# GBATZOLIS/conditional_score_diffusion

Measured on AMD Instinct MI355X. Metric: images/sec for 1000-step PC sampling, ddpm_paired_SR3 score net of celebA_SR3_160 (BASELINE configs[1]), 160x160, higher is better.
Workload: dtype f16x3 (every operand carried as hi + lo fp16 = 22 significand bits, 3 MFMAs per product, f32 accumulate; f32-class: the per-op test tolerance is the f32 kernel's, network error 1.9e-6 vs the reference); 1 GPU; BASELINE configs[1]: celebA_SR3_160 (ddpm_paired_SR3, nf=96, ch_mult (1,1,2,2,3,3), attn 20/10/5), 1000-step PC (reverse_diffusion + langevin, snr 0.15), batch 64 per GPU, random-init weights, synthetic LR inputs; images_per_gpu=64, global_batch=64, noise=on-device Philox4x32-10, precision_mode=fp16x3

## Files before the change

### conditional_score_diffusion_amd/csrc/conv_f16_q.hip

```cpp
#include <stdlib.h>
#include <type_traits>

#include "conv_f16_kernel.h"

namespace csd {

typedef float floatx4q __attribute__((ext_vector_type(4)));
typedef unsigned int uint4q __attribute__((ext_vector_type(4)));

#define C16Q_THREADS 256

__device__ __forceinline__ double dpp_row16_sum(double v) {
#define CSD_DPP_STEP(CTRL)                                                                                   \
  {                                                                                                          \
    const int lo = __builtin_amdgcn_mov_dpp(__double2loint(v), CTRL, 0xF, 0xF, true);                        \
    const int hi = __builtin_amdgcn_mov_dpp(__double2hiint(v), CTRL, 0xF, 0xF, true);                        \
    v += __hiloint2double(hi, lo);                                                                           \
  }
  CSD_DPP_STEP(0xB1)
  CSD_DPP_STEP(0x4E)
  CSD_DPP_STEP(0x124)
  CSD_DPP_STEP(0x128)
#undef CSD_DPP_STEP
  return v;
}
__device__ __forceinline__ float dpp_row16_sum(float v) {
#define CSD_DPP_STEP_F(CTRL) v += __int_as_float(__builtin_amdgcn_mov_dpp(__float_as_int(v), CTRL, 0xF, 0xF, true));
  CSD_DPP_STEP_F(0xB1)
  CSD_DPP_STEP_F(0x4E)
  CSD_DPP_STEP_F(0x124)
  CSD_DPP_STEP_F(0x128)
#undef CSD_DPP_STEP_F
  return v;
}

typedef int int8q __attribute__((ext_vector_type(8)));

template <int MQ, int NS, bool MASK, int PWC, int S, int NTQ, bool F8, bool UP4 = false, bool RAW = false>
__global__ __launch_bounds__(C16Q_THREADS, 2) void conv_f16_q_kernel(const void* __restrict__ g_hi,
                                                                    const void* __restrict__ g_lo,
                                                                    const char* __restrict__ g_wpack,
                                                                    const Conv16KArgs k) {
  static_assert(!UP4 || (S == 1 && !F8), "the phase form is the stride-1 Upsample conv (a resampling conv: full split)");
  static_assert(!RAW || (NS == 2 && !F8), "the fp32-source form splits into two fp16 planes");
  constexpr int TAPS = UP4 ? 4 : 9, KS = UP4 ? 2 : 3, KCS = 2;
  constexpr int LO = 32 * KCS;
  constexpr int PSB = 32 * KCS * NS + 16;
  constexpr int NPIX = 2 * MQ * 16;
  constexpr int SPP = 2 * NS * KCS;
  constexpr int NU0 = (S == 2) ? ((NS == 2) ? 10 : 5) : ((NS == 2) ? 7 : 4);
  constexpr int NU = RAW ? 2 * ((NU0 + 1) / 2) : NU0;
  constexpr int rstride = PWC * PSB;
  constexpr int WSTEP = NTQ * NS * 1024;
  constexpr int GC = 32 * NTQ, HC = 16 * NTQ;
  extern __shared__ __attribute__((aligned(16))) char smem16[];

  const int tid = threadIdx.x;
#ifdef CSD_C16_TIMING
  int ts_n = 0;
#define Q_TSTAMP() do { if (k.a.dbg && tid == 0 && blockIdx.x < 4095 && ts_n < 8) k.a.dbg[blockIdx.x * 8 + ts_n++] = clock64(); } while (0)
#else
#define Q_TSTAMP() do { } while (0)
#endif
  Q_TSTAMP();
  const int lane = tid & 63;
  const int wave = __builtin_amdgcn_readfirstlane(tid >> 6);
  const int mi = wave >> 1, ni = wave & 1;
  const int l16 = lane & 15, kq = lane >> 4;

  int w;
  {
    const int bid = blockIdx.x, nb = k.nblocks;
    const int xcd = bid & 7, slot = bid >> 3;
    const int q = nb >> 3, r = nb & 7;
    w = (xcd < r ? xcd * (q + 1) : r * (q + 1) + (xcd - r) * q) + slot;
  }
  const int ng = w % k.n_groups;
  const int tile4 = w / k.n_groups;
  const int ph = UP4 ? (tile4 & 3) : 0, pa = ph >> 1, pb = ph & 1;
  const int tile = UP4 ? (tile4 >> 2) : tile4;
  const int tile_y = tile / k.tiles_x;
  const int ov0 = tile_y * k.TH, ox0 = (tile - tile_y * k.tiles_x) * k.TW;
  const int Py = UP4 ? 1 - pa : ((S == 2) ? 0 : 1), Px = UP4 ? 1 - pb : ((S == 2) ? 0 : 1);
  const int prow0 = ov0 * S - Py, pcol0 = ox0 * S - Px;
  const int EH = (S == 2) ? k.IH : k.OH, EW = (S == 2) ? k.IW : k.OW;
  const int Cin = k.C0;
  const int npatch = k.PH * k.PW;
  const int patch_bytes = k.PH * PWC * PSB;
  int* const otab = reinterpret_cast<int*>(smem16 + patch_bytes);
  int* const btab = otab + NPIX;
  int* const vtab = btab + NPIX;
  int* const stab = vtab + NPIX;
  int* const dtab = stab + npatch;

  for (int m = tid; m < NPIX; m += C16Q_THREADS) {
    const int ty = m / k.TW, tx = m - ty * k.TW;
    const int ov = ov0 + ty, ox = ox0 + tx;
    const bool mv = (m < k.TH * k.TW) && (ov < k.B * k.OH) && (ox < k.OW);
    const int b = ov / k.OH, oy = ov - b * k.OH;
    unsigned vb = 0;
#pragma unroll
    for (int r = 0; r < KS; ++r) {
      const int iy = oy * S + r - Py, ix = ox * S + r - Px;
      vb |= ((mv && iy >= 0 && iy < EH) ? 1u : 0u) << r;
      vb |= ((mv && ix >= 0 && ix < EW) ? 1u : 0u) << (3 + r);
    }
    otab[m] = mv ? (UP4 ? (ov - ov0) * 4 * k.OW + 2 * ox : (ov - ov0) * k.OW + ox) : -1;
    btab[m] = mv ? b : 0;
    vtab[m] = (int)vb;
  }
  for (int pix = tid; pix < npatch; pix += C16Q_THREADS) {
    const int pr = pix / k.PW, pc = pix - pr * k.PW;
    const int vr = prow0 + pr, col = pcol0 + pc;
    const int img_lo = MASK ? 0 : (ov0 / k.OH) * EH;
    const int img_hi = MASK ? k.B * EH : img_lo + EH;
    const bool in = vr >= img_lo && vr < img_hi && col >= 0 && col < EW;
    const int sb = vr / EH, sr = vr - sb * EH;
    stab[pix] = in ? (sb * k.IH + (sr >> k.up)) * k.IW + (col >> k.up) : -1;
    dtab[pix] = (pr * PWC + pc) * PSB;
  }
  int base[MQ];
#pragma unroll
  for (int j = 0; j < MQ; ++j) {
    const int m = (mi * MQ + j) * 16 + l16;
    const int ty = m / k.TW, tx = m - ty * k.TW;
    base[j] = (m < k.TH * k.TW) ? ty * S * rstride + tx * S * PSB + kq * 16 : kq * 16;
  }
  __syncthreads();
  Q_TSTAMP();
  unsigned vbits[MQ];
  if (MASK) {
#pragma unroll
    for (int j = 0; j < MQ; ++j) vbits[j] = (unsigned)vtab[(mi * MQ + j) * 16 + l16];
  }

  const int total4 = RAW ? npatch * 2 * KCS : npatch * SPP;
  auto raw_load = [&](int e, int cb, int half) -> float4 {
    float4 v = make_float4(0.f, 0.f, 0.f, 0.f);
    if (e < total4) {
      const int pix = e / (2 * KCS), grp = e - pix * (2 * KCS);
      const int sp = stab[pix];
      if (sp >= 0) v = gload4f(static_cast<const float*>(g_hi) + (size_t)sp * Cin + cb + grp * 8 + half * 4);
    }
    return v;
  };
  auto raw_store = [&](int e, const float4& a, const float4& b) {
    if (e >= total4) return;
    const int pix = e / (2 * KCS), grp = e - pix * (2 * KCS);
    const float v[8] = {a.x, a.y, a.z, a.w, b.x, b.y, b.z, b.w};
    half8 h, l;
#pragma unroll
    for (int j = 0; j < 8; ++j) {
      h[j] = (_Float16)v[j];
      l[j] = (_Float16)(v[j] - (float)h[j]);
    }
    *reinterpret_cast<half8*>(smem16 + dtab[pix] + grp * 16) = h;
    *reinterpret_cast<half8*>(smem16 + dtab[pix] + LO + grp * 16) = l;
  };
  auto slot_load = [&](int e, int cb) -> float4 {
    float4 v = make_float4(0.f, 0.f, 0.f, 0.f);
    if (e < total4) {
      const int pix = e / SPP, sub = e - pix * SPP;
      const int sp = stab[pix];
      if (sp >= 0) {
        const int pl = sub / (2 * KCS), rest = sub - pl * (2 * KCS);
        const _Float16* plane = static_cast<const _Float16*>((NS == 2 && pl) ? g_lo : g_hi);
        v = gload4f(reinterpret_cast<const float*>(plane + (size_t)sp * Cin + cb + rest * 8));
      }
    }
    return v;
  };
  auto slot_store = [&](int e, const float4& v) {
    if (e >= total4) return;
    const int pix = e / SPP, sub = e - pix * SPP;
    const int pl = sub / (2 * KCS), rest = sub - pl * (2 * KCS);
    *reinterpret_cast<float4*>(smem16 + dtab[pix] + pl * LO + rest * 16) = v;
  };

  constexpr int BR = UP4 ? 2 : (NTQ == 1 && !F8 ? 9 : 3);
  const int nk32 = Cin / 32;
  const char* wstep = g_wpack + ((size_t)((UP4 ? ph * k.n_groups * 2 : 0) + ng * 2 + ni) * nk32 * TAPS) * WSTEP + lane * 16;
  constexpr int NP = F8 ? 1 : NS;
  half8 wreg[BR][NTQ][NP];
#pragma unroll
  for (int q = 0; q < BR - 1; ++q)
#pragma unroll
    for (int t = 0; t < NTQ; ++t)
#pragma unroll
      for (int p = 0; p < NP; ++p) wreg[q][t][p] = gload_h8(wstep + (size_t)q * WSTEP + (t * NS + p) * 1024);
  wstep += (size_t)(BR - 2) * WSTEP;
  const char* const w8base = g_wpack + ((size_t)(ng * 2 + ni) * nk32 * TAPS + (kq >> 1)) * WSTEP + (lane & 31) * 32 + 1024;
  int8q w8[1][NTQ];
  auto load_w8 = [&](int buf, int step) {
#pragma unroll
    for (int t = 0; t < NTQ; ++t) {
      const uint4q a = *reinterpret_cast<const uint4q*>(w8base + (size_t)step * WSTEP + t * NS * 1024);
      const uint4q c = *reinterpret_cast<const uint4q*>(w8base + (size_t)step * WSTEP + t * NS * 1024 + 16);
      w8[buf][t] = int8q{(int)a.x, (int)a.y, (int)a.z, (int)a.w, (int)c.x, (int)c.y, (int)c.z, (int)c.w};
    }
  };
  if constexpr (F8) load_w8(0, 0);
  int base8[MQ];
#pragma unroll
  for (int j = 0; j < MQ; ++j) base8[j] = base[j] - kq * 16 + LO + (kq & 1) * 32;

  floatx4q acc[MQ][NTQ];
#pragma unroll
  for (int j = 0; j < MQ; ++j)
#pragma unroll
    for (int t = 0; t < NTQ; ++t) acc[j][t] = floatx4q{0.f, 0.f, 0.f, 0.f};

  {
    float4 v0[NU];
    if constexpr (RAW) {
#pragma unroll
      for (int j = 0; j < NU; ++j) v0[j] = raw_load((j >> 1) * C16Q_THREADS + tid, 0, j & 1);
#pragma unroll
      for (int j = 0; j < NU; j += 2) raw_store((j >> 1) * C16Q_THREADS + tid, v0[j], v0[j + 1]);
    } else {
#pragma unroll
      for (int j = 0; j < NU; ++j) v0[j] = slot_load(j * C16Q_THREADS + tid, 0);
#pragma unroll
      for (int j = 0; j < NU; ++j) slot_store(j * C16Q_THREADS + tid, v0[j]);
    }
  }
  __syncthreads();
  Q_TSTAMP();

  const int nstage = nk32;
  for (int stg = 0; stg < nstage; ++stg) {
    const bool more = stg + 1 < nstage;
    float4 sv[NU];
    if (more) {
#pragma unroll
      for (int j = 0; j < NU; ++j)
        sv[j] = RAW ? raw_load((j >> 1) * C16Q_THREADS + tid, (stg + 1) * 32, j & 1) : slot_load(j * C16Q_THREADS + tid, (stg + 1) * 32);
    }
#ifdef CSD_Q_RING
    constexpr int RING = CSD_Q_RING;
#else
    constexpr int RING = 2;
#endif
    half8 preg[RING][NP];
    auto load_frag = [&](int q) {
      const int tap_ = q / MQ, j_ = q % MQ;
      const char* p = smem16 + base[j_] + (tap_ / KS) * rstride + (tap_ % KS) * PSB;
#pragma unroll
      for (int pl = 0; pl < NP; ++pl) preg[q % RING][pl] = *reinterpret_cast<const half8*>(p + pl * LO);
    };
#pragma unroll
    for (int q = 0; q < RING - 1; ++q) load_frag(q);
#pragma unroll
    for (int tap = 0; tap < TAPS; ++tap) {
      const int bc = tap % BR, bn = (tap + BR - 1) % BR;
      const int r = tap / KS, sx = tap % KS;
      wstep += WSTEP;
#ifndef CSD_Q_ABLATE
#define CSD_Q_ABLATE 0
#endif
#pragma unroll
      for (int t = 0; t < ((CSD_Q_ABLATE & 1) ? 1 : NTQ); ++t)
#pragma unroll
        for (int p = 0; p < NP; ++p) wreg[bn][t][p] = gload_h8(wstep + (t * NS + p) * 1024);

#pragma unroll
      for (int j = 0; j < MQ; ++j) {
        const int q = tap * MQ + j;
        if (q + RING - 1 < TAPS * MQ) load_frag(q + RING - 1);
        __builtin_amdgcn_sched_barrier(0);
        half8 b[NP];
        const bool v = !MASK || (((vbits[j] >> r) & 1u) && ((vbits[j] >> (3 + sx)) & 1u));
#pragma unroll
        for (int pl = 0; pl < NP; ++pl) {
          b[pl] = preg[q % RING][pl];
          if (MASK && !v) {
#pragma unroll
            for (int e = 0; e < 8; ++e) b[pl][e] = (_Float16)0.f;
          }
        }
#pragma unroll
        for (int t = 0; t < NTQ; ++t) {
          if constexpr (NS == 2 && !F8) {
            acc[j][t] = __builtin_amdgcn_mfma_f32_16x16x32_f16(wreg[bc][t][1], b[0], acc[j][t], 0, 0, 0);
            acc[j][t] = __builtin_amdgcn_mfma_f32_16x16x32_f16(wreg[bc][t][0], b[1], acc[j][t], 0, 0, 0);
          }
          acc[j][t] = __builtin_amdgcn_mfma_f32_16x16x32_f16(wreg[bc][t][0], b[0], acc[j][t], 0, 0, 0);
        }
        __builtin_amdgcn_sched_barrier(0);
      }
      if constexpr (F8) {
        if (tap % 2 == 1 || tap == TAPS - 1) {
          const int t0 = tap % 2 == 1 ? tap - 1 : tap;
          const bool pair = t0 + 1 < TAPS;
          const int t1 = pair ? t0 + 1 : t0;
          const int o0 = (t0 / KS) * rstride + (t0 % KS) * PSB, o1 = (t1 / KS) * rstride + (t1 % KS) * PSB;
          const int off = (kq >> 1) ? o1 : o0;
          constexpr int wb = 0;
#pragma unroll
          for (int j = 0; j < MQ; ++j) {
            const char* xp = smem16 + base8[j] + off;
            const uint4q a = *reinterpret_cast<const uint4q*>(xp);
            const uint4q c = *reinterpret_cast<const uint4q*>(xp + 16);
            bool ok = pair || (kq >> 1) == 0;
            if (MASK) {
              const int tt = (kq >> 1) ? t1 : t0;
              ok = ok && ((vbits[j] >> (tt / KS)) & 1u) && ((vbits[j] >> (3 + tt % KS)) & 1u);
            }
            const int8q b8 = int8q{ok ? (int)a.x : 0, ok ? (int)a.y : 0, ok ? (int)a.z : 0, ok ? (int)a.w : 0,
                                   ok ? (int)c.x : 0, ok ? (int)c.y : 0, ok ? (int)c.z : 0, ok ? (int)c.w : 0};
#pragma unroll
            for (int t = 0; t < NTQ; ++t)
              acc[j][t] = __builtin_amdgcn_mfma_scale_f32_16x16x128_f8f6f4(w8[wb][t], b8, acc[j][t], 0, 0, 0, 116, 0, 127);
          }
          const int nxt = t0 + 2 < TAPS ? stg * TAPS + t0 + 2 : (stg + 1) * TAPS;
          if (t0 + 2 < TAPS || more) load_w8(0, nxt);
        }
      }
    }
    static_assert(TAPS % BR == 0, "weight ring phase");
    Q_TSTAMP();
    if (more) {
      __syncthreads();
      if constexpr (RAW) {
#pragma unroll
        for (int j = 0; j < NU; j += 2) raw_store((j >> 1) * C16Q_THREADS + tid, sv[j], sv[j + 1]);
      } else {
#pragma unroll
        for (int j = 0; j < NU; ++j) slot_store(j * C16Q_THREADS + tid, sv[j]);
      }
      __syncthreads();
    }
  }

  constexpr unsigned OOB = 0x80000000u;
  constexpr int RSRC_FLAGS = 0x00020000;
  const float wunscale = 1.0f / C16_WSCALE;
  const size_t o_base = UP4 ? ((size_t)(2 * ov0 + pa) * 2 * k.OW + pb) : (size_t)ov0 * k.OW;
  const int b0 = ov0 / k.OH;
  const bool has_res = k.a.res != nullptr, has_temb = k.a.temb != nullptr;
  const __amdgpu_buffer_rsrc_t out_r =
      __builtin_amdgcn_make_buffer_rsrc(k.a.out + o_base * k.a.out_stride + k.a.out_coff, 0, OOB, RSRC_FLAGS);
  const __amdgpu_buffer_rsrc_t res_r = __builtin_amdgcn_make_buffer_rsrc(
      const_cast<float*>(has_res ? k.a.res + o_base * k.Cout : k.a.out), 0, OOB, RSRC_FLAGS);
  const int c_base = ng * GC + ni * HC + kq * 4;
  int oidx[MQ];
#pragma unroll
  for (int j = 0; j < MQ; ++j) oidx[j] = otab[(mi * MQ + j) * 16 + l16];
  float4 bias4[NTQ], tvu4[NTQ];
#pragma unroll
  for (int t = 0; t < NTQ; ++t) {
    const int c0 = c_base + t * 16;
    bias4[t] = k.a.bias ? gload4f(k.a.bias + c0) : make_float4(0.f, 0.f, 0.f, 0.f);
    tvu4[t] = (!MASK && has_temb) ? gload4f(k.a.temb + (size_t)b0 * k.a.temb_stride + c0) : make_float4(0.f, 0.f, 0.f, 0.f);
  }
  float4 addv[MQ][NTQ];
#pragma unroll
  for (int j = 0; j < MQ; ++j)
#pragma unroll
    for (int t = 0; t < NTQ; ++t) {
      float4 a = tvu4[t];
      if (has_res) {
        const unsigned off = oidx[j] >= 0 ? (unsigned)(oidx[j] * k.Cout + c_base + t * 16) * 4u : OOB;
        const uint4q rv = __builtin_amdgcn_raw_buffer_load_b128(res_r, off, 0, 0);
        const float4 rr = make_float4(__uint_as_float(rv.x), __uint_as_float(rv.y), __uint_as_float(rv.z), __uint_as_float(rv.w));
        a = (MASK || !has_temb) ? rr : make_float4(rr.x + a.x, rr.y + a.y, rr.z + a.z, rr.w + a.w);
      }
      addv[j][t] = a;
    }
  if (MASK && has_temb) {
#pragma unroll
    for (int j = 0; j < MQ; ++j) {
      const int b = btab[(mi * MQ + j) * 16 + l16];
#pragma unroll
      for (int t = 0; t < NTQ; ++t) {
        const float4 tv = gload4f(k.a.temb + (size_t)b * k.a.temb_stride + c_base + t * 16);
        addv[j][t] = make_float4(addv[j][t].x + tv.x, addv[j][t].y + tv.y, addv[j][t].z + tv.z, addv[j][t].w + tv.w);
      }
    }
  }
  using st_t = typename std::conditional<UP4, float, double>::type;
  st_t st_s[NTQ][4], st_q[NTQ][4];
#pragma unroll
  for (int t = 0; t < NTQ; ++t)
#pragma unroll
    for (int i = 0; i < 4; ++i) { st_s[t][i] = 0; st_q[t][i] = 0; }
#pragma unroll
  for (int j = 0; j < MQ; ++j)
#pragma unroll
    for (int t = 0; t < NTQ; ++t) {
      const float b4[4] = {bias4[t].x, bias4[t].y, bias4[t].z, bias4[t].w};
      const float a4[4] = {addv[j][t].x, addv[j][t].y, addv[j][t].z, addv[j][t].w};
      float o4[4];
#pragma unroll
      for (int i = 0; i < 4; ++i) {
        o4[i] = ((acc[j][t][i] * wunscale + b4[i]) + a4[i]) * k.a.out_scale;
        const st_t dv = oidx[j] >= 0 ? (st_t)o4[i] : (st_t)0;
        st_s[t][i] += dv;
        st_q[t][i] = fma(dv, dv, st_q[t][i]);
      }
      uint4q ov;
      ov.x = __float_as_uint(o4[0]); ov.y = __float_as_uint(o4[1]); ov.z = __float_as_uint(o4[2]); ov.w = __float_as_uint(o4[3]);
      const unsigned off = oidx[j] >= 0 ? (unsigned)(oidx[j] * k.a.out_stride + c_base + t * 16) * 4u : OOB;
      __builtin_amdgcn_raw_buffer_store_b128(ov, out_r, off, 0, 0);
    }
  if (k.a.stats) {
#pragma unroll
    for (int t = 0; t < NTQ; ++t)
#pragma unroll
      for (int i = 0; i < 4; ++i) {
        const double s = (double)dpp_row16_sum(st_s[t][i]), q = (double)dpp_row16_sum(st_q[t][i]);
        if (l16 == 0)
          *reinterpret_cast<double2*>(k.a.stats + (((size_t)tile4 * 2 + mi) * k.Cout + c_base + t * 16 + i) * 2) = make_double2(s, q);
      }
  }
  Q_TSTAMP();
}

bool conv16q_supported(const ConvPlan& p, int ns) {
  return (ns >= 1 && ns <= 3) && p.taps == 9 && ((p.stride == 1 && (p.up == 0 || p.up == 1)) || (p.stride == 2 && p.up == 0)) &&
         p.C1 == 0 && p.C0 % 32 == 0 &&
         (p.qnt == 1 ? (p.Cout % 32 == 0 && ns >= 2 && p.stride == 1 && p.up == 0) : (p.Cout % 96 == 0 || (p.Cout % 128 == 0 && ns != 3)));
}

bool conv16q_up4_stats_ok(const ConvPlan& p) { return p.up == 2 && (long)p.IH * p.IW >= 1600 && p.IH % p.TH == 0; }

bool conv16q_up4_supported(const ConvPlan& p, int ns) {
  ConvPlan q = p;
  q.up = 1;
  return (ns == 1 || ns == 2) && p.stride == 1 && conv16q_supported(q, ns) && !CSD_TUNE_ENV("CSD_NO_UP4");
}

size_t conv16q_up4_packed_bytes(const ConvPlan& p, int ns) {
  const int ntq = p.Cout % 96 == 0 ? 3 : 4;
  return (size_t)4 * (p.Cout / (32 * ntq)) * 2 * (p.C0 / 32) * 4 * ntq * ns * 1024 + (size_t)4 * ntq * ns * 1024;
}

__global__ void conv16q_pack_up4_kernel(const float* __restrict__ w, _Float16* __restrict__ wpack, int Cin, int Cout, int ns, int ntq) {
  const size_t idx = (size_t)blockIdx.x * blockDim.x + threadIdx.x;
  const size_t total = (size_t)Cout * Cin * 16;
  {
    const size_t body32 = (size_t)4 * (Cout / (32 * ntq)) * 2 * (Cin / 32) * 4 * ntq * ns * 256, slack32 = (size_t)ntq * ns * 1024;
    if (idx < slack32) reinterpret_cast<uint32_t*>(wpack)[body32 + idx] = 0u;
  }
  if (idx >= total) return;
  const int pt = (int)(idx % 16), ph = pt >> 2, tap = pt & 3;
  const int cin = (int)((idx / 16) % Cin);
  const int cout = (int)(idx / ((size_t)16 * Cin));
  const int a = ph >> 1, b = ph & 1, i = tap >> 1, j = tap & 1;
  const int r0 = a == 0 ? (i == 0 ? 0 : 1) : (i == 0 ? 0 : 2), r1 = a == 0 ? (i == 0 ? 0 : 2) : (i == 0 ? 1 : 2);
  const int s0 = b == 0 ? (j == 0 ? 0 : 1) : (j == 0 ? 0 : 2), s1 = b == 0 ? (j == 0 ? 0 : 2) : (j == 0 ? 1 : 2);
  float v = 0.f;
  for (int r = r0; r <= r1; ++r)
    for (int sx = s0; sx <= s1; ++sx) v += w[((size_t)cout * Cin + cin) * 9 + r * 3 + sx];
  v *= C16_WSCALE;
  const int gc = 32 * ntq, hc = 16 * ntq;
  const int ng = cout / gc, ni = (cout % gc) / hc, t = (cout % hc) / 16, rr = cout % 16;
  const int kb = cin / 32, kq = (cin % 32) / 8, q = cin % 8;
  const int lane = kq * 16 + rr;
  const size_t step = (((size_t)ph * (Cout / gc) * 2 + ng * 2 + ni) * (Cin / 32) + kb) * 4 + tap;
  _Float16* dst = wpack + (step * ntq + t) * (size_t)ns * 512 + lane * 8 + q;
  const _Float16 hi = (_Float16)v;
  dst[0] = hi;
  if (ns == 2) dst[512] = (_Float16)(v - (float)hi);
}

int conv16q_pack_weight_up4(const ConvPlan& p, int ns, const float* w, void* wpack, hipStream_t s) {
  const size_t total = (size_t)p.Cout * p.C0 * 16;
  hipLaunchKernelGGL(conv16q_pack_up4_kernel, dim3((unsigned)cdiv64(total, 256)), dim3(256), 0, s, w, (_Float16*)wpack, p.C0, p.Cout, ns,
                     p.Cout % 96 == 0 ? 3 : 4);
  CSD_LAUNCH_CHECK();
  return CSD_OK;
}

static inline int q_ntq(const ConvPlan& p) { return p.qnt ? p.qnt : (p.Cout % 96 == 0 ? 3 : 4); }

size_t conv16q_packed_bytes(const ConvPlan& p, int ns) {
  if (ns == 3) ns = 2;
  const int ntq = q_ntq(p);
  return (size_t)(p.Cout / (32 * ntq)) * 2 * (p.C0 / 32) * 9 * ntq * ns * 1024 + (size_t)8 * ntq * ns * 1024;
}

__global__ void conv16q_pack_kernel(const float* __restrict__ w, _Float16* __restrict__ wpack, int layout, int cin_src,
                                    int cout_src, int cout_off, int Cin, int Cout, int ns, int ntq, int f8) {
  const size_t idx = (size_t)blockIdx.x * blockDim.x + threadIdx.x;
  const size_t total = (size_t)cout_src * Cin * 9;
  if (idx >= total) return;
  {
    const size_t body32 = (size_t)(Cout / (32 * ntq)) * 2 * (Cin / 32) * 9 * ntq * ns * 256, slack32 = (size_t)2 * ntq * ns * 1024;
    if (cout_off == 0 && idx < slack32) reinterpret_cast<uint32_t*>(wpack)[body32 + idx] = 0u;
  }
  const int tap = (int)(idx % 9);
  const int cin = (int)((idx / 9) % Cin);
  const int co = (int)(idx / ((size_t)9 * Cin));
  const int cout = cout_off + co;
  if (cin >= cin_src || cout >= Cout) return;
  const float v = ((layout == 0) ? w[((size_t)co * cin_src + cin) * 9 + tap]
                   : (layout == 1) ? w[(size_t)cin * cout_src + co]
                                   : w[((size_t)cin * cout_src + co) * 9 + (8 - tap)]) * C16_WSCALE;
  const int gc = 32 * ntq, hc = 16 * ntq;
  const int ng = cout / gc, ni = (cout % gc) / hc, t = (cout % hc) / 16, r = cout % 16;
  const int kb = cin / 32, kq = (cin % 32) / 8, q = cin % 8;
  const int lane = kq * 16 + r;
  const size_t step = ((size_t)(ng * 2 + ni) * (Cin / 32) + kb) * 9 + tap;
  _Float16* dst = wpack + (step * ntq + t) * (size_t)ns * 512 + lane * 8 + q;
  const _Float16 hi = (_Float16)v;
  dst[0] = hi;
  if (ns == 2 && !f8) dst[512] = (_Float16)(v - (float)hi);
  if (f8) {
    const float hf = fminf(fmaxf((float)hi, -448.f), 448.f), lf = fminf(fmaxf((v - (float)hi) * 2048.f, -448.f), 448.f);
    const int pk = __builtin_amdgcn_cvt_pk_fp8_f32(hf, lf, 0, false);
    unsigned char* c8 = reinterpret_cast<unsigned char*>(wpack + ((step * ntq + t) * (size_t)ns + 1) * 512) +
                        (((cin % 32) / 16) * 16 + r) * 32 + (cin % 16) * 2;
    c8[0] = (unsigned char)(pk & 255);
    c8[1] = (unsigned char)((pk >> 8) & 255);
  }
}

__global__ void conv16q_zero_kernel(uint32_t* p, size_t n) {
  const size_t i = (size_t)blockIdx.x * blockDim.x + threadIdx.x;
  if (i < n) p[i] = 0u;
}

int conv16q_pack_weight(const ConvPlan& p, int ns, const float* w, int layout, int cin_src, int cout_src, int cout_off,
                        void* wpack, hipStream_t s) {
  const int f8 = ns == 3;
  if (f8) ns = 2;
  if (cout_off == 0 && (cin_src != p.C0 || cout_src != p.Cout)) {
    const size_t n32 = conv16q_packed_bytes(p, ns) / 4;
    hipLaunchKernelGGL(conv16q_zero_kernel, dim3((unsigned)cdiv64(n32, 256)), dim3(256), 0, s, (uint32_t*)wpack, n32);
    CSD_LAUNCH_CHECK();
  }
  const size_t total = (size_t)cout_src * p.C0 * 9;
  hipLaunchKernelGGL(conv16q_pack_kernel, dim3((unsigned)cdiv64(total, 256)), dim3(256), 0, s, w, (_Float16*)wpack, layout,
                     cin_src, cout_src, cout_off, p.C0, p.Cout, ns, q_ntq(p), f8);
  CSD_LAUNCH_CHECK();
  return CSD_OK;
}

static int in_coord_q(int t, int stride = 1) { return stride * (t - 1) + 3; }
static int in_coord_k(int t, int stride, int ks) { return stride * (t - 1) + ks; }

int conv16q_plan_tiles(ConvPlan* p, int ns) {
  const bool up4 = p->up == 2;
  CSD_REQUIRE(up4 ? conv16q_up4_supported(*p, ns) : conv16q_supported(*p, ns), "conv16q: unsupported shape (Cin=%d Cout=%d)", p->C0, p->Cout);
  const int OHt = up4 ? p->IH : p->OH, OWt = up4 ? p->IW : p->OW, ks = up4 ? 2 : 3;
  p->KC = C16_KC;
  p->CoutPad = p->Cout;
  p->NT = q_ntq(*p);
  p->n_groups = p->Cout / (32 * p->NT);
  p->KCS = 2;
  p->LC = 0;
  if (ns == 3) ns = 2;
  const int psb = 32 * 2 * ns + 16;
  const int spp = 2 * ns * 2;
  const int st = p->stride;
  const int nu = st == 2 ? (ns == 2 ? 10 : 5) : (ns == 2 ? 7 : 4);
  auto pitch = [&](int tw) { return in_coord_k(tw, st, ks) <= 24 ? 24 : 34; };
  int best_mq = 0, best_tw = 0, best_th = 0;
  for (int mq = p->qnt == 1 ? 2 : 4; mq >= 2; mq >>= 1) {
    const int npix = 2 * mq * 16;
    int btw = 0, bth = 0, blds = 1 << 30;
    double bcov = -1;
    bool bunm = false;
    for (int tw = 1; tw <= 32 && tw <= OWt; ++tw) {
      if (OWt % tw != 0 && !(tw == 32 && OWt > 32)) continue;
      if (in_coord_k(tw, st, ks) > 34) continue;
      for (int th = npix / tw; th >= 1; --th) {
        const int patch = in_coord_k(th, st, ks) * in_coord_k(tw, st, ks);
        const int lds = in_coord_k(th, st, ks) * pitch(tw) * psb;
        if (lds > 72 * 1024 || patch * spp > nu * C16Q_THREADS) continue;
        const double cov = (double)th * tw * OWt / ((double)cdiv(OWt, tw) * tw);
        const bool unm = (OHt % th) == 0;
        if (cov > bcov + 1e-9 || (cov > bcov - 1e-9 && ((unm && !bunm) || (unm == bunm && lds < blds)))) {
          bcov = cov; blds = lds; btw = tw; bth = th; bunm = unm;
        }
        break;
      }
    }
    if (btw == 0) continue;
    if (mq > 2 && bcov < 0.75 * npix) continue;
    best_mq = mq; best_tw = btw; best_th = bth;
    const long nwg = (long)cdiv(OWt, btw) * cdiv(p->B * OHt, bth) * p->n_groups * (up4 ? 4 : 1);
    static const long min_wg = CSD_TUNE_ENV("CSD_Q_MINWG") ? atol(CSD_TUNE_ENV("CSD_Q_MINWG")) : 300;
    if (up4 && (long)OHt * OWt >= 1600) break;
    if (nwg >= min_wg || mq == 2) break;
  }
  CSD_REQUIRE(best_tw > 0, "conv16q: no feasible tile for OW=%d", p->OW);
  p->TW = best_tw; p->TH = best_th;
  p->PH = in_coord_k(p->TH, st, ks); p->PW = in_coord_k(p->TW, st, ks);
  p->tiles_x = cdiv(OWt, p->TW);
  p->tiles_y = cdiv(p->B * OHt, p->TH);
  p->MT = best_mq;
  p->lds_bytes = (size_t)p->PH * pitch(p->TW) * psb + (size_t)3 * 2 * best_mq * 16 * sizeof(int) +
                 (size_t)2 * p->PH * p->PW * sizeof(int);
  return CSD_OK;
}

template <int MQ, int NS, bool MASK, int PWC, int S, int NTQ, bool F8 = false, bool UP4 = false, bool RAW = false>
static int launch_q(const Conv16KArgs& k, size_t lds, hipStream_t s) {
  auto kern = conv_f16_q_kernel<MQ, NS, MASK, PWC, S, NTQ, F8, UP4, RAW>;
  static bool attr_set = false;
  if (!attr_set) {
    CSD_CHECK_HIP(hipFuncSetAttribute(reinterpret_cast<const void*>(kern), hipFuncAttributeMaxDynamicSharedMemorySize, 160 * 1024));
    attr_set = true;
  }
  hipLaunchKernelGGL(kern, dim3(k.nblocks), dim3(C16Q_THREADS), lds, s, static_cast<const void*>(k.a.src0),
                     static_cast<const void*>(k.a.src1), reinterpret_cast<const char*>(k.a.wpack), k);
  CSD_LAUNCH_CHECK();
  return CSD_OK;
}

template <int MQ, int NS, bool MASK, int PWC, int S, int NTQ, bool UP4>
static int launch_q_src(bool raw, const Conv16KArgs& k, size_t lds, hipStream_t s) {
  if constexpr (NS == 2 && NTQ >= 3) {
    if (raw) return launch_q<MQ, NS, MASK, PWC, S, NTQ, false, UP4, true>(k, lds, s);
  }
  if (raw) {
    set_error("conv16q: no fp32-source kernel for ns=%d NT=%d", NS, NTQ);
    return CSD_ERR_INVALID;
  }
  return launch_q<MQ, NS, MASK, PWC, S, NTQ, false, UP4, false>(k, lds, s);
}

int conv16q_launch(const ConvPlan& p, int ns, const ConvArgs& a, hipStream_t s, bool raw) {
  const bool up4 = p.up == 2;
  CSD_REQUIRE(up4 ? conv16q_up4_supported(p, ns) : conv16q_supported(p, ns), "conv16q: unsupported layer");
  CSD_REQUIRE(!a.out_nchw && a.nscale == nullptr && a.out_stride % 4 == 0 && a.out_coff % 4 == 0,
              "conv16q: NHWC fp32 output with 16-byte aligned rows, pre-normalised fp16 source");
  Conv16KArgs k;
  k.a = a;
  k.a.dbg = nullptr;
#ifdef CSD_C16_TIMING
  {
    extern long long* g_c16_dbg; extern int g_c16_dbg_blocks, g_c16_dbg_max, g_c16_dbg_n;
    const int nb = cdiv(p.OW, p.TW) * cdiv(p.B * p.OH, p.TH) * p.n_groups;
    if (g_c16_dbg && nb == g_c16_dbg_blocks && g_c16_dbg_n < g_c16_dbg_max) {
      k.a.dbg = g_c16_dbg + (size_t)g_c16_dbg_n * 4096 * 8;
      if (hipMemsetAsync(k.a.dbg, 0, 4096 * 8 * 8, s) != hipSuccess) return -1;
      long long hdr[4] = {p.C0, p.Cout, 1, (a.res ? 1 : 0) | (a.temb ? 2 : 0)};
      if (hipMemcpyAsync(k.a.dbg + 4095 * 8, hdr, sizeof(hdr), hipMemcpyHostToDevice, s) != hipSuccess) return -1;
      g_c16_dbg_n++;
    }
  }
#endif
  k.B = p.B; k.IH = p.IH; k.IW = p.IW; k.OH = p.OH; k.OW = p.OW;
  k.C0 = p.C0; k.C1 = 0; k.Cout = p.Cout;
  k.stride = p.stride; k.pad = p.stride == 2 ? 0 : 1; k.up = p.up;
  k.TH = p.TH; k.TW = p.TW; k.PH = p.PH; k.PW = p.PW;
  k.tiles_x = p.tiles_x; k.n_groups = p.n_groups;
  k.nblocks = p.tiles_x * p.tiles_y * p.n_groups * (up4 ? 4 : 1);
  if (up4) { k.OH = p.IH; k.OW = p.IW; k.up = 0; }
  k.nck = p.C0 / C16_KC;
  k.nw = 4;
  k.ntiles_n = p.Cout / 32;
  const bool mask = ((up4 ? p.IH : p.OH) % p.TH) != 0;
#define CSD_QU_CASE(MQ_, NS_, NTQ_)                                                              \
  if (up4 && p.MT == MQ_ && ns == NS_ && p.NT == NTQ_) {                                        \
    if (p.PW <= 24) {                                                                            \
      if (mask) return launch_q_src<MQ_, NS_, true, 24, 1, NTQ_, true>(raw, k, p.lds_bytes, s);    \
      return launch_q_src<MQ_, NS_, false, 24, 1, NTQ_, true>(raw, k, p.lds_bytes, s);             \
    }                                                                                            \
    if (mask) return launch_q_src<MQ_, NS_, true, 34, 1, NTQ_, true>(raw, k, p.lds_bytes, s);      \
    return launch_q_src<MQ_, NS_, false, 34, 1, NTQ_, true>(raw, k, p.lds_bytes, s);               \
  }
  CSD_QU_CASE(4, 2, 3) CSD_QU_CASE(2, 2, 3) CSD_QU_CASE(4, 1, 3) CSD_QU_CASE(2, 1, 3)
  CSD_QU_CASE(4, 2, 4) CSD_QU_CASE(2, 2, 4) CSD_QU_CASE(4, 1, 4) CSD_QU_CASE(2, 1, 4)
#undef CSD_QU_CASE
  CSD_REQUIRE(!up4, "conv16q: no phase kernel for MQ=%d ns=%d NT=%d", p.MT, ns, p.NT);
#define CSD_Q_CASE(MQ_, NS_, NTQ_)                                                  \
  if (p.MT == MQ_ && ns == NS_ && p.NT == NTQ_ && p.stride == 1) {                  \
    if (p.PW <= 24) {                                                               \
      if (mask) return launch_q_src<MQ_, NS_, true, 24, 1, NTQ_, false>(raw, k, p.lds_bytes, s);    \
      return launch_q_src<MQ_, NS_, false, 24, 1, NTQ_, false>(raw, k, p.lds_bytes, s);             \
    }                                                                               \
    if (mask) return launch_q_src<MQ_, NS_, true, 34, 1, NTQ_, false>(raw, k, p.lds_bytes, s);      \
    return launch_q_src<MQ_, NS_, false, 34, 1, NTQ_, false>(raw, k, p.lds_bytes, s);               \
  }                                                                                 \
  if (p.MT == MQ_ && ns == NS_ && p.NT == NTQ_ && p.stride == 2) {                  \
    if (p.PW <= 24) {                                                               \
      if (mask) return launch_q_src<MQ_, NS_, true, 24, 2, NTQ_, false>(raw, k, p.lds_bytes, s);    \
      return launch_q_src<MQ_, NS_, false, 24, 2, NTQ_, false>(raw, k, p.lds_bytes, s);             \
    }                                                                               \
    if (mask) return launch_q_src<MQ_, NS_, true, 34, 2, NTQ_, false>(raw, k, p.lds_bytes, s);      \
    return launch_q_src<MQ_, NS_, false, 34, 2, NTQ_, false>(raw, k, p.lds_bytes, s);               \
  }
#define CSD_Q8_CASE(MQ_, NTQ_)                                                         \
  if (p.MT == MQ_ && ns == 3 && p.NT == NTQ_ && p.stride == 1) {                     \
    if (p.PW <= 24) {                                                                \
      if (mask) return launch_q<MQ_, 2, true, 24, 1, NTQ_, true>(k, p.lds_bytes, s);  \
      return launch_q<MQ_, 2, false, 24, 1, NTQ_, true>(k, p.lds_bytes, s);           \
    }                                                                                \
    if (mask) return launch_q<MQ_, 2, true, 34, 1, NTQ_, true>(k, p.lds_bytes, s);    \
    return launch_q<MQ_, 2, false, 34, 1, NTQ_, true>(k, p.lds_bytes, s);             \
  }                                                                                  \
  if (p.MT == MQ_ && ns == 3 && p.NT == NTQ_ && p.stride == 2) {                     \
    if (p.PW <= 24) {                                                                \
      if (mask) return launch_q<MQ_, 2, true, 24, 2, NTQ_, true>(k, p.lds_bytes, s);  \
      return launch_q<MQ_, 2, false, 24, 2, NTQ_, true>(k, p.lds_bytes, s);           \
    }                                                                                \
    if (mask) return launch_q<MQ_, 2, true, 34, 2, NTQ_, true>(k, p.lds_bytes, s);    \
    return launch_q<MQ_, 2, false, 34, 2, NTQ_, true>(k, p.lds_bytes, s);             \
  }
  CSD_REQUIRE(!(raw && ns == 3), "conv16q: the fp8-correction form reads pre-split planes");
  CSD_Q8_CASE(4, 3) CSD_Q8_CASE(2, 3) CSD_Q8_CASE(2, 1)
#undef CSD_Q8_CASE
  CSD_Q_CASE(4, 2, 3) CSD_Q_CASE(2, 2, 3) CSD_Q_CASE(4, 1, 3) CSD_Q_CASE(2, 1, 3) CSD_Q_CASE(2, 2, 1)
  CSD_Q_CASE(4, 2, 4) CSD_Q_CASE(2, 2, 4) CSD_Q_CASE(4, 1, 4) CSD_Q_CASE(2, 1, 4)
#undef CSD_Q_CASE
  set_error("conv16q: no kernel for MQ=%d ns=%d NT=%d", p.MT, ns, p.NT);
  return CSD_ERR_INVALID;
}

}
```

Before: 1.634 images/sec.

## Deepen input-patch prefetch to multiple stages and precompute per-thread slot tables

Replaces the single-stage register prefetch of input patch data with a D-deep (default 3) ring of in-flight global loads for the common MQ==2 stride-1 configuration, so more K-stages of activations are outstanding while MFMAs run. Per-thread slot addresses (source pixel and smem destination with zero/dead flags) are computed once and kept in registers instead of being re-derived with divisions every stage. Out-of-range loads are clamped to valid addresses and zeroed at deposit time, and the epilogue recomputes lane indices to reduce live registers. This raises register pressure and may lower occupancy, which the TABREG guard tries to limit for heavy configurations.

```diff
diff --git a/conditional_score_diffusion_amd/csrc/conv_f16_q.hip b/conditional_score_diffusion_amd/csrc/conv_f16_q.hip
--- a/conditional_score_diffusion_amd/csrc/conv_f16_q.hip
+++ b/conditional_score_diffusion_amd/csrc/conv_f16_q.hip
@@ -85,6 +85,7 @@
   const int prow0 = ov0 * S - Py, pcol0 = ox0 * S - Px;
   const int EH = (S == 2) ? k.IH : k.OH, EW = (S == 2) ? k.IW : k.OW;
   const int Cin = k.C0;
+  const int nk32 = Cin / 32;
   const int npatch = k.PH * k.PW;
   const int patch_bytes = k.PH * PWC * PSB;
   int* const otab = reinterpret_cast<int*>(smem16 + patch_bytes);
@@ -134,51 +135,78 @@
     for (int j = 0; j < MQ; ++j) vbits[j] = (unsigned)vtab[(mi * MQ + j) * 16 + l16];
   }
 
-  const int total4 = RAW ? npatch * 2 * KCS : npatch * SPP;
-  auto raw_load = [&](int e, int cb, int half) -> float4 {
-    float4 v = make_float4(0.f, 0.f, 0.f, 0.f);
-    if (e < total4) {
-      const int pix = e / (2 * KCS), grp = e - pix * (2 * KCS);
-      const int sp = stab[pix];
-      if (sp >= 0) v = gload4f(static_cast<const float*>(g_hi) + (size_t)sp * Cin + cb + grp * 8 + half * 4);
-    }
-    return v;
+  constexpr int NSL = RAW ? NU / 2 : NU;
+  constexpr int EPP = RAW ? 2 * KCS : SPP;
+  constexpr unsigned SLOT_ZERO = 0x80000000u, SLOT_DEAD = 0x40000000u, SLOT_OFF = 0x00FFFFFFu;
+  constexpr unsigned SPARE = 32 * KCS * NS;
+  static_assert(C16Q_THREADS % EPP == 0, "a thread's slots share their place inside the pixel");
+  const int sub_t = tid % EPP, pix_t = tid / EPP;
+  const int pl_t = RAW ? 0 : sub_t / (2 * KCS), rest_t = RAW ? sub_t : sub_t - pl_t * (2 * KCS);
+  const char* const src_t = reinterpret_cast<const char*>(static_cast<const _Float16*>((NS == 2 && pl_t) ? g_lo : g_hi) + rest_t * 8);
+  auto slot_of = [&](int j, int& sp, unsigned& off) {
+    const int pix = pix_t + j * (C16Q_THREADS / EPP);
+    const bool live = pix < npatch;
+    const int cpix = live ? pix : 0;
+    const int s = stab[cpix];
+    sp = (live && s >= 0) ? s : 0;
+    off = live ? ((unsigned)(dtab[cpix] + pl_t * LO + rest_t * 16) | (s < 0 ? SLOT_ZERO : 0u)) : (SPARE | SLOT_DEAD);
   };
-  auto raw_store = [&](int e, const float4& a, const float4& b) {
-    if (e >= total4) return;
-    const int pix = e / (2 * KCS), grp = e - pix * (2 * KCS);
-    const float v[8] = {a.x, a.y, a.z, a.w, b.x, b.y, b.z, b.w};
-    half8 h, l;
-#pragma unroll
-    for (int j = 0; j < 8; ++j) {
-      h[j] = (_Float16)v[j];
-      l[j] = (_Float16)(v[j] - (float)h[j]);
-    }
-    *reinterpret_cast<half8*>(smem16 + dtab[pix] + grp * 16) = h;
-    *reinterpret_cast<half8*>(smem16 + dtab[pix] + LO + grp * 16) = l;
+#ifndef CSD_Q_TABREG
+#define CSD_Q_TABREG 1
+#endif
+  constexpr bool TABREG = CSD_Q_TABREG && !(MQ == 4 && NS == 2 && (F8 || NTQ == 4));
+  int ssp[TABREG ? NSL : 1];
+  unsigned sdo[TABREG ? NSL : 1];
+  if constexpr (TABREG) {
+#pragma unroll
+    for (int j = 0; j < NSL; ++j) slot_of(j, ssp[j], sdo[j]);
+  }
+  auto slot_get = [&](int j, int& sp, unsigned& off) {
+    if constexpr (TABREG) { sp = ssp[j]; off = sdo[j]; } else slot_of(j, sp, off);
   };
-  auto slot_load = [&](int e, int cb) -> float4 {
-    float4 v = make_float4(0.f, 0.f, 0.f, 0.f);
-    if (e < total4) {
-      const int pix = e / SPP, sub = e - pix * SPP;
-      const int sp = stab[pix];
-      if (sp >= 0) {
-        const int pl = sub / (2 * KCS), rest = sub - pl * (2 * KCS);
-        const _Float16* plane = static_cast<const _Float16*>((NS == 2 && pl) ? g_lo : g_hi);
-        v = gload4f(reinterpret_cast<const float*>(plane + (size_t)sp * Cin + cb + rest * 8));
-      }
-    }
-    return v;
+  auto request = [&](float4 (&set)[NU], int stg) {
+    const bool past = stg >= nk32;
+    const int cb = past ? 0 : stg * 32;
+    const int pitch = past ? 0 : Cin;
+#pragma unroll
+    for (int j = 0; j < NSL; ++j) {
+      int sp; unsigned off;
+      slot_get(j, sp, off);
+      if constexpr (RAW) {
+        const float* p = static_cast<const float*>(g_hi) + ((size_t)sp * pitch + cb + rest_t * 8);
+        set[2 * j] = gload4f(p);
+        set[2 * j + 1] = gload4f(p + 4);
+      } else {
+        set[j] = gload4f(reinterpret_cast<const float*>(src_t + ((size_t)sp * pitch + cb) * 2));
+      }
+    }
   };
-  auto slot_store = [&](int e, const float4& v) {
-    if (e >= total4) return;
-    const int pix = e / SPP, sub = e - pix * SPP;
-    const int pl = sub / (2 * KCS), rest = sub - pl * (2 * KCS);
-    *reinterpret_cast<float4*>(smem16 + dtab[pix] + pl * LO + rest * 16) = v;
+  auto zero_if = [](bool z, const float4& v) { return make_float4(z ? 0.f : v.x, z ? 0.f : v.y, z ? 0.f : v.z, z ? 0.f : v.w); };
+  auto deposit = [&](const float4 (&set)[NU]) {
+#pragma unroll
+    for (int j = 0; j < NSL; ++j) {
+      int sp; unsigned off;
+      slot_get(j, sp, off);
+      const bool z = (off & SLOT_ZERO) != 0;
+      char* const dst = smem16 + (off & SLOT_OFF);
+      if constexpr (RAW) {
+        const float4 a = zero_if(z, set[2 * j]), b = zero_if(z, set[2 * j + 1]);
+        const float v[8] = {a.x, a.y, a.z, a.w, b.x, b.y, b.z, b.w};
+        half8 h, l;
+#pragma unroll
+        for (int i = 0; i < 8; ++i) {
+          h[i] = (_Float16)v[i];
+          l[i] = (_Float16)(v[i] - (float)h[i]);
+        }
+        *reinterpret_cast<half8*>(dst) = h;
+        *reinterpret_cast<half8*>(dst + ((off & SLOT_DEAD) ? 0 : LO)) = l;
+      } else {
+        *reinterpret_cast<float4*>(dst) = zero_if(z, set[j]);
+      }
+    }
   };
 
   constexpr int BR = UP4 ? 2 : (NTQ == 1 && !F8 ? 9 : 3);
-  const int nk32 = Cin / 32;
   const char* wstep = g_wpack + ((size_t)((UP4 ? ph * k.n_groups * 2 : 0) + ng * 2 + ni) * nk32 * TAPS) * WSTEP + lane * 16;
   constexpr int NP = F8 ? 1 : NS;
   half8 wreg[BR][NTQ][NP];
@@ -210,32 +238,25 @@
 #pragma unroll
     for (int t = 0; t < NTQ; ++t) acc[j][t] = floatx4q{0.f, 0.f, 0.f, 0.f};
 
-  {
-    float4 v0[NU];
-    if constexpr (RAW) {
-#pragma unroll
-      for (int j = 0; j < NU; ++j) v0[j] = raw_load((j >> 1) * C16Q_THREADS + tid, 0, j & 1);
-#pragma unroll
-      for (int j = 0; j < NU; j += 2) raw_store((j >> 1) * C16Q_THREADS + tid, v0[j], v0[j + 1]);
-    } else {
-#pragma unroll
-      for (int j = 0; j < NU; ++j) v0[j] = slot_load(j * C16Q_THREADS + tid, 0);
-#pragma unroll
-      for (int j = 0; j < NU; ++j) slot_store(j * C16Q_THREADS + tid, v0[j]);
-    }
-  }
+#ifndef CSD_Q_DEPTH
+#define CSD_Q_DEPTH 3
+#endif
+  constexpr int D = (MQ == 2 && S == 1 && !RAW && !F8 && !UP4 && NTQ <= 3) ? CSD_Q_DEPTH : 1;
+  float4 sv[D][NU];
+#pragma unroll
+  for (int d = 0; d < D; ++d) request(sv[d], d);
+  deposit(sv[0]);
   __syncthreads();
   Q_TSTAMP();
 
   const int nstage = nk32;
-  for (int stg = 0; stg < nstage; ++stg) {
+  for (int stg0 = 0; stg0 < nstage; stg0 += D) {
+#pragma unroll
+   for (int d = 0; d < D; ++d) {
+    const int stg = stg0 + d;
+    if (d > 0 && stg >= nstage) break;
     const bool more = stg + 1 < nstage;
-    float4 sv[NU];
-    if (more) {
-#pragma unroll
-      for (int j = 0; j < NU; ++j)
-        sv[j] = RAW ? raw_load((j >> 1) * C16Q_THREADS + tid, (stg + 1) * 32, j & 1) : slot_load(j * C16Q_THREADS + tid, (stg + 1) * 32);
-    }
+    request(sv[d], stg + D);
 #ifdef CSD_Q_RING
     constexpr int RING = CSD_Q_RING;
 #else
@@ -313,7 +334,7 @@
               acc[j][t] = __builtin_amdgcn_mfma_scale_f32_16x16x128_f8f6f4(w8[wb][t], b8, acc[j][t], 0, 0, 0, 116, 0, 127);
           }
           const int nxt = t0 + 2 < TAPS ? stg * TAPS + t0 + 2 : (stg + 1) * TAPS;
-          if (t0 + 2 < TAPS || more) load_w8(0, nxt);
+          load_w8(0, nxt);
         }
       }
     }
@@ -321,17 +342,18 @@
     Q_TSTAMP();
     if (more) {
       __syncthreads();
-      if constexpr (RAW) {
-#pragma unroll
-        for (int j = 0; j < NU; j += 2) raw_store((j >> 1) * C16Q_THREADS + tid, sv[j], sv[j + 1]);
-      } else {
-#pragma unroll
-        for (int j = 0; j < NU; ++j) slot_store(j * C16Q_THREADS + tid, sv[j]);
-      }
+      deposit(sv[(d + 1) % D]);
       __syncthreads();
     }
-  }
-
+   }
+  }
+#pragma unroll
+  for (int d = 0; d < D; ++d)
+#pragma unroll
+    for (int j = 0; j < NU; ++j) asm volatile("" ::"v"(sv[d][j].x), "v"(sv[d][j].y), "v"(sv[d][j].z), "v"(sv[d][j].w));
+
+  const int lane_e = __builtin_amdgcn_mbcnt_hi(~0u, __builtin_amdgcn_mbcnt_lo(~0u, 0u));
+  const int l16e = lane_e & 15, kqe = lane_e >> 4;
   constexpr unsigned OOB = 0x80000000u;
   constexpr int RSRC_FLAGS = 0x00020000;
   const float wunscale = 1.0f / C16_WSCALE;
@@ -342,10 +364,10 @@
       __builtin_amdgcn_make_buffer_rsrc(k.a.out + o_base * k.a.out_stride + k.a.out_coff, 0, OOB, RSRC_FLAGS);
   const __amdgpu_buffer_rsrc_t res_r = __builtin_amdgcn_make_buffer_rsrc(
       const_cast<float*>(has_res ? k.a.res + o_base * k.Cout : k.a.out), 0, OOB, RSRC_FLAGS);
-  const int c_base = ng * GC + ni * HC + kq * 4;
+  const int c_base = ng * GC + ni * HC + kqe * 4;
   int oidx[MQ];
 #pragma unroll
-  for (int j = 0; j < MQ; ++j) oidx[j] = otab[(mi * MQ + j) * 16 + l16];
+  for (int j = 0; j < MQ; ++j) oidx[j] = otab[(mi * MQ + j) * 16 + l16e];
   float4 bias4[NTQ], tvu4[NTQ];
 #pragma unroll
   for (int t = 0; t < NTQ; ++t) {
@@ -370,7 +392,7 @@
   if (MASK && has_temb) {
 #pragma unroll
     for (int j = 0; j < MQ; ++j) {
-      const int b = btab[(mi * MQ + j) * 16 + l16];
+      const int b = btab[(mi * MQ + j) * 16 + l16e];
 #pragma unroll
       for (int t = 0; t < NTQ; ++t) {
         const float4 tv = gload4f(k.a.temb + (size_t)b * k.a.temb_stride + c_base + t * 16);
@@ -409,7 +431,7 @@
 #pragma unroll
       for (int i = 0; i < 4; ++i) {
         const double s = (double)dpp_row16_sum(st_s[t][i]), q = (double)dpp_row16_sum(st_q[t][i]);
-        if (l16 == 0)
+        if (l16e == 0)
           *reinterpret_cast<double2*>(k.a.stats + (((size_t)tile4 * 2 + mi) * k.Cout + c_base + t * 16 + i) * 2) = make_double2(s, q);
       }
   }
```

Measured after the change: 1.640 images/sec, median of 6. About the same (+0.4%).
